# Wenyuan-Vincent-Li/Tensorflow-Implementation-of-Triple-GAN

Measured on AMD Instinct MI355X. Metric: Triple-GAN train images/sec (G+C+D step) CIFAR-10 32x32 bs=100, higher is better.
Workload: dtype f32; 1 GPU; CIFAR-10 32x32x3, 4000 labelled, bs=100 fp32 (B_G/L_C/U_C/L_D/U_D=100/50/50/20/80), Good_GAN_cifar10 D+G+C step; global_batch=100, parallelism=dp1, exec_mode=auto, exec_mode_chosen=plan, hip_graph=False

## Files before the change

### include/tg_kernels.h

```cpp
#ifndef TG_KERNELS_H
#define TG_KERNELS_H

#include <stdint.h>

#ifdef __cplusplus
extern "C" {
#endif

typedef enum tg_status {
  TG_OK = 0,
  TG_ERR_INVALID = -1,
  TG_ERR_HIP = -2,
  TG_ERR_STATE = -3
} tg_status;

enum { TG_ACT_NONE = 0, TG_ACT_LRELU = 1, TG_ACT_RELU = 2, TG_ACT_TANH = 3, TG_ACT_SIGMOID = 4, TG_ACT_SOFTPLUS = 5 };

int tg_version(void);
const char* tg_last_error_string(void);
int tg_device_count(void);

int tg_graph_begin_capture(void* stream);
int tg_graph_end_capture(void* stream, void** graph_exec_out);
int tg_graph_launch(void* graph_exec, void* stream);
// ... 71 lines not shown

int tg_conv3x3_packed_supported(int n, int h, int w, int c_in, int c_out);
int64_t tg_conv3x3_packed_wgrad_workspace_bytes(int n, int h, int w, int c_in, int c_out);
int tg_conv3x3_packed_fwd_f32(const float* x, int ld_x, int c_in, const float* kernel, const float* bias, int act, float alpha, const float* labels,
                              int lab_n, float* y, int ld_y, int n, int h, int w, int c_out, void* stream);
int tg_conv3x3_packed_wgrad_f32(const float* x, int ld_x, int c_in, const float* dy, int ld_dy, int n, int h, int w, int c_out, float* workspace,
                                float* dw, void* stream);

int tg_deconv5x5s2_narrow_supported(int n, int h, int w, int c_out, int ci_p);
int64_t tg_deconv5x5s2_narrow_wgrad_workspace_bytes(int n, int h, int w, int c_out, int ci_p);
int tg_deconv5x5s2_narrow_dgrad_f32(const float* dy, int ld_dy, const float* kernel, const float* scale_a, int n, int h, int w, int c_out, int c_in,
                                    int ci_p, float* dx, int ld_dx, void* stream);
int tg_deconv5x5s2_narrow_wgrad_f32(const float* dy, int ld_dy, const float* x, int ld_x, int n, int h, int w, int c_out, int c_in, int ci_p,
                                    float* workspace, float* dw, void* stream);

int tg_conv2d_desc_fwd(int n, int h, int w, int ld_in, int c_out, int k, int stride, int pad_same, int ld_out, int n_store, int act, float alpha,
                       tg_igemm_desc* d);
int tg_conv2d_desc_dgrad(int n, int h, int w, int c_in_pad, int ld_dy, int k, int stride, int pad_same, int ld_out, int n_store, tg_igemm_desc* descs,
                         int32_t* n_desc_out);
int tg_conv2d_desc_wgrad(int n, int h, int w, int ld_in, int c_out_pad, int k, int stride, int pad_same, int ld_dy, tg_igemm_desc* d);
int tg_deconv5x5s2_desc_fwd(int n, int h, int w, int ld_in, int c_out_pad, int ld_out, int n_store, int act, tg_igemm_desc* descs, int32_t* n_desc_out);
int tg_deconv5x5s2_desc_fwd_merged(int n, int h, int w, int ld_in, int c_out, int ld_out, int n_store, int act, tg_igemm_desc* d, int32_t* n_group_out,
                                   int32_t* tapmap);
int tg_deconv5x5s2_desc_dgrad(int n, int h, int w, int c_in_pad, int ld_dy, int ld_out, int n_store, tg_igemm_desc* d);
int tg_deconv5x5s2_desc_wgrad(int n, int h, int w, int ld_dy, int c_in_pad, int ld_x, tg_igemm_desc* d);
int tg_dense_desc(int m, int ld_in, int c_out, int ld_out, int n_store, int act, int64_t w_sn, tg_igemm_desc* d);
int tg_dense_splitk_desc(int m, int k_dim, int n_out, int splits, tg_igemm_desc* descs);
int tg_wgrad_splits(const tg_igemm_desc* d);
int tg_wgrad_splits_bf16(const tg_igemm_desc* d);
int64_t tg_wgrad_workspace_bytes(const tg_igemm_desc* d, int n_split);
int64_t tg_filter_workspace_bytes(int n_taps, int c_in_pad, int c_out_pad);
int tg_igemm_tile(const tg_igemm_desc* descs, int n_desc, const int32_t* seg_rows, int nseg, int bf16, int32_t* bm_out, int32_t* bn_out);
int tg_igemm_colsum_supported(const tg_igemm_desc* d, const int32_t* seg_rows, int nseg);
int tg_wgrad_tile(const tg_igemm_desc* d, int32_t* ct_out, int32_t* nt_out);

int tg_conv3x3_policy(int policy);
int64_t tg_conv3x3_launches(void);

int tg_wn_scale_f32(const float* v, const float* g, int rows, int c, float* scale, void* stream);

int tg_filter_prep_f32(const float* src, const float* scale, const float* scale_a, int t, int a, int b, int a_pad, int b_pad, float* dst_same,
                       float* dst_tr, int64_t tr_sb, int64_t tr_st, void* stream);

int tg_wn_scale_tab_f32(const float* v, const float* g, int t, int a, int b, float* scale_a, void* stream);
int tg_wn_bwd_tab_f32(const float* dw, const float* v, const float* g, int t, int a, int b, float* dv, float* dg, void* stream);

int tg_deconv_merge_prep_f32(const float* w, const float* scale_a, int c_out, int c_in, int n_group, int n_pad, int c_pad,
                             const int32_t* tapmap, float* dst, void* stream);
typedef struct tg_prep_job {
  const float* src;
  const float* g;
  float* scale;
  float* dst_same;
  float* dst_tr;
  int64_t tr_sb, tr_st;
  int32_t t, a, b, a_pad, b_pad;
} tg_prep_job;
int tg_filter_prep_multi_f32(const tg_prep_job* jobs, int n_jobs, void* stream);
typedef struct tg_wn_job {
  const float* slab;
  float* dw;
  const float* v;
  const float* g;
  float* dv;
  float* dg;
  float* coef;
// ... 181 lines not shown
```

### tensorflow-implementation-of-triple-gan_amd/csrc/geom.cpp

```cpp
#include <cstring>

#include "tg_common.h"
#include "tg_geom.h"
#include "tg_conv3x3_bf16.h"

namespace {

inline int pad32(int c) { return (c + 31) / 32 * 32; }

struct Pad { int out, before; };

Pad same_pad(int n, int k, int s) {
  const int out = (n + s - 1) / s;
  int total = (out - 1) * s + k - n;
  if (total < 0) total = 0;
  return {out, total / 2};
}

Pad out_size(int n, int k, int s, int pad_same) { return pad_same ? same_pad(n, k, s) : Pad{(n - k) / s + 1, 0}; }

struct Tap { int dy, dx, tw; };

int fill(tg_igemm_desc* d, int n_img, int h_in, int w_in, int ld_in, int h_v, int w_v, int s, int h_out, int w_out, int ld_out, int os, int oo_y,
         int oo_x, int c_out, int n_store, const Tap* taps, int n_taps, int64_t w_sn, int64_t w_st, int act, float alpha) {
// ... 88 lines not shown
    int shortest = nk[0];
    for (int s = 1; s < n_sub; ++s) shortest = nk[s] < shortest ? nk[s] : shortest;
    for (;;) {
      int longest = 0, ls = -1, sum = 0;
      for (int s = 0; s < n_sub; ++s) {
        sum += best_ks[s];
        const int len = (nk[s] + best_ks[s] - 1) / best_ks[s];
        if (len > longest) { longest = len; ls = s; }
      }
      if (ls < 0 || best_ks[ls] >= 4 || T * (sum + 1) > slots || sum + 1 > 16) break;
      if (nk[ls] / (best_ks[ls] + 1) < mink || longest * 4 <= shortest * 5) break;
      ++best_ks[ls];
    }
  }
  int len = 0, nslot = 0, nsp = 0;
  for (int s = 0; s < n_sub; ++s) {
    o->ks[s] = best_ks[s];
    if (best_ks[s] > 1) { o->split_sub[nsp] = (int8_t)s; o->first_slot[nsp] = (int8_t)nslot; ++nsp; }
    for (int k = 0; k < best_ks[s]; ++k) {
      o->pat_sub[len] = (int8_t)s; o->pat_k[len] = (int8_t)k;
      o->pat_slot[len] = best_ks[s] > 1 ? (int8_t)nslot++ : (int8_t)-1;
      ++len;
    }
  }
  o->pat_len = len;
  o->n_pat_split = nslot;
  o->n_split_sub = nsp;
  o->nfull = (int)T;
  o->n_units = (int)(T * len);
  o->n_fix = (int)(T * nsp);
  o->ws_bytes = T * nslot * (int64_t)bm * bn * 4;
}

int wgrad_tile(int n) { return n % 128 == 0 ? 128 : ((n % 64 == 0 || n >= 160) ? 64 : 32); }

}

extern "C" {

int tg_conv2d_desc_fwd(int n, int h, int w, int ld_in, int c_out, int k, int stride, int pad_same, int ld_out, int n_store, int act, float alpha,
                       tg_igemm_desc* d) {
  GEOM_ARGS_OK(d && n > 0 && h > 0 && w > 0 && k >= 1 && k <= 5 && stride >= 1 && (pad_same || (h >= k && w >= k)), "conv2d_desc_fwd: bad arguments");
  const Pad py = out_size(h, k, stride, pad_same), px = out_size(w, k, stride, pad_same);
  Tap taps[TG_MAX_TAPS];
  int nt = 0;
  for (int ky = 0; ky < k; ++ky)
    for (int kx = 0; kx < k; ++kx) taps[nt++] = {ky - py.before, kx - px.before, ky * k + kx};
  if (ld_out <= 0) ld_out = c_out;
  if (n_store < 0) n_store = c_out;
  return fill(d, n, h, w, ld_in, py.out, px.out, stride, py.out, px.out, ld_out, 1, 0, 0, c_out, n_store, taps, nt, (int64_t)k * k * ld_in, ld_in, act, alpha);
}

int tg_conv2d_desc_dgrad(int n, int h, int w, int c_in_pad, int ld_dy, int k, int stride, int pad_same, int ld_out, int n_store, tg_igemm_desc* descs,
                         int32_t* n_desc_out) {
  GEOM_ARGS_OK(descs && n_desc_out && n > 0 && h > 0 && w > 0 && k >= 1 && k <= 5 && stride >= 1 && stride <= 2, "conv2d_desc_dgrad: bad arguments");
  const Pad py = out_size(h, k, stride, pad_same), px = out_size(w, k, stride, pad_same);
  if (ld_out <= 0) ld_out = c_in_pad;
  if (n_store < 0) n_store = c_in_pad;
  int nd = 0;
  for (int qy = 0; qy < stride; ++qy)
    for (int qx = 0; qx < stride; ++qx) {
      Tap taps[TG_MAX_TAPS];
      int nt = 0;
      for (int ky = 0; ky < k; ++ky) {
        if (((qy + py.before - ky) % stride + stride) % stride) continue;
        for (int kx = 0; kx < k; ++kx) {
// ... 114 lines not shown
  const int ct = tg::wgrad_tile(d->ld_in), nt = tg::wgrad_tile(d->c_out);
  const int64_t tiles = (int64_t)d->n_taps * ((d->ld_in + ct - 1) / ct) * ((d->c_out + nt - 1) / nt);
  const int64_t m = (int64_t)d->n_img * d->h_v * d->w_v;
  int64_t ns = 512 / tiles;
  if (ns > m / 128) ns = m / 128;
  return (int)(ns < 1 ? 1 : ns);
}

int tg_wgrad_splits_bf16(const tg_igemm_desc* d) {
  if (!d || d->ld_in <= 0 || d->c_out <= 0 || d->n_taps <= 0) { tg::set_error("wgrad_splits_bf16: bad descriptor"); return TG_ERR_INVALID; }
  const int ns = tg::wgrad3x3_splits(d, true, tg::halo_policy(), tg::halo_compute_units());
  return ns > 0 ? ns : tg_wgrad_splits(d);
}

int64_t tg_wgrad_workspace_bytes(const tg_igemm_desc* d, int n_split) {
  if (!d || n_split < 1) { tg::set_error("wgrad_workspace_bytes: bad arguments"); return TG_ERR_INVALID; }
  return (int64_t)n_split * d->n_taps * d->ld_in * d->c_out * 4;
}

int64_t tg_filter_workspace_bytes(int n_taps, int c_in_pad, int c_out_pad) {
  if (n_taps < 1 || c_in_pad < 1 || c_out_pad < 1) { tg::set_error("filter_workspace_bytes: bad arguments"); return TG_ERR_INVALID; }
  return (int64_t)n_taps * c_in_pad * c_out_pad * 4;
}

int tg_igemm_tile(const tg_igemm_desc* descs, int n_desc, const int32_t* seg_rows, int nseg, int bf16, int32_t* bm_out, int32_t* bn_out) {
  TG_REQUIRE(descs && n_desc >= 1 && n_desc <= 4 && bm_out && bn_out, "igemm_tile: bad arguments");
  int bm = 0, bn = 0;
  TG_REQUIRE(tg::igemm_pick_tile(descs, n_desc, nseg > 0, seg_rows, nseg, bf16 != 0, &bm, &bn), "igemm_tile: no tile fits c_out=%d with the given segments",
             descs[0].c_out);
  *bm_out = bm; *bn_out = bn;
  return TG_OK;
}

int tg_wgrad_tile(const tg_igemm_desc* d, int32_t* ct_out, int32_t* nt_out) {
  TG_REQUIRE(d && ct_out && nt_out && d->ld_in > 0 && d->c_out > 0, "wgrad_tile: bad arguments");
  *ct_out = tg::wgrad_tile(d->ld_in);
  *nt_out = tg::wgrad_tile(d->c_out);
  return TG_OK;
}

int tg_igemm_colsum_supported(const tg_igemm_desc* d, const int32_t* seg_rows, int nseg) {
  if (!d || !seg_rows || nseg < 1 || nseg > 8 || d->n_group != 0) return 0;
  int64_t tot = 0;
  for (int i = 0; i < nseg; ++i) { if (seg_rows[i] < 32) return 0; tot += seg_rows[i]; }
  if (tot != (int64_t)d->n_img * d->h_v * d->w_v) return 0;
  int bm, bn;
  return tg::igemm_pick_tile(d, 1, true, seg_rows, nseg, false, &bm, &bn) ? 1 : 0;
}

}
```

### tensorflow-implementation-of-triple-gan_amd/csrc/igemm.hip

```cpp
#include <cstdio>
#include <cstring>
#include "tg_common.h"
#include "tg_device.h"
#include "tg_geom.h"
#include "tg_conv3x3_bf16.h"

typedef float f32x4 __attribute__((ext_vector_type(4)));
typedef float f32x16 __attribute__((ext_vector_type(16)));
typedef __bf16 bf16x8 __attribute__((ext_vector_type(8)));

namespace {

__device__ __forceinline__ bf16x8 cvt8(f32x4 lo, f32x4 hi) {
  bf16x8 r;
  r[0] = (__bf16)lo[0]; r[1] = (__bf16)lo[1]; r[2] = (__bf16)lo[2]; r[3] = (__bf16)lo[3];
  r[4] = (__bf16)hi[0]; r[5] = (__bf16)hi[1]; r[6] = (__bf16)hi[2]; r[7] = (__bf16)hi[3];
  return r;
}

typedef short s16x4 __attribute__((ext_vector_type(4)));
typedef __bf16 bf16x4_t __attribute__((ext_vector_type(4)));
typedef unsigned int u32x2 __attribute__((ext_vector_type(2)));
typedef unsigned int u32x4 __attribute__((ext_vector_type(4)));

// ... 26 lines not shown
  float alpha;
  int32_t n_group;
  int32_t taps[TG_MAX_TAPS];
};

struct IgemmParams {
  const float* in;
  const float* w;
  const float* bias;
  float* out;
  SubDesc d[MAX_SUB];
  int64_t w_sn, w_st;
  int n_img, h_in, w_in, ld_in, c_out;
  int n_sub, M, m_tiles, n_tiles;
  uint32_t in_bytes, w_bytes, out_bytes;
  double* colsum;
  const float* ymul;
  int ymul_act;
  float ymul_alpha;
  int stat2;
  int nseg, seg_rows[8];
  const float* lab;
  int lab_n, lab_c0;
  int n_units;
  int n_fix;
  int nfull;
  int ks[MAX_SUB];
  int pat_len;
  int n_pat_split;
  int n_split_sub;
  int8_t pat_sub[16], pat_k[16], pat_slot[16];
  int8_t split_sub[MAX_SUB], first_slot[MAX_SUB];
  float* ws;
};


__device__ __forceinline__ float apply_act(float v, int act, float alpha) {
  switch (act) {
    case TG_ACT_LRELU: return v > 0.f ? v : alpha * v;
    case TG_ACT_RELU: return v > 0.f ? v : 0.f;
    case TG_ACT_TANH: return tanhf(v);
    case TG_ACT_SIGMOID: return 1.f / (1.f + __expf(-v));
    case TG_ACT_SOFTPLUS: return v > 20.f ? v : log1pf(__expf(v));
    default: return v;
  }
}

__device__ __forceinline__ int xcd_remap(int bid, int nwg) {
  const int q = nwg >> 3, r = nwg & 7, x = bid & 7;
  return (x < r ? x * (q + 1) : r * (q + 1) + (x - r) * q) + (bid >> 3);
}

template <int BM, int BN, int WAVES_M, int WAVES_N, bool COLSUM, bool BF16, bool FIXUP = false>
__global__ void __launch_bounds__(256, 2) igemm_f32_kernel(IgemmParams p) {
  static_assert(WAVES_M * WAVES_N == 4, "4 waves");
  constexpr int WM = BM / WAVES_M, WN = BN / WAVES_N, MI = WM / 32, NI = WN / 32;
  constexpr int AR = BM / 32, BR = BN / 32;
  constexpr int NBUF = 2;
  constexpr int PF = FIXUP ? 1 : (BM * BN >= 128 * 128 ? 1 : 2);
  __shared__ __attribute__((aligned(16))) float smem[NBUF * BM * LDT + NBUF * BN * LDT + 4 * BM];
  float* As = smem;
  float* Bs = smem + NBUF * BM * LDT;
  int* t_base = reinterpret_cast<int*>(smem + NBUF * BM * LDT + NBUF * BN * LDT);
  int* t_y = t_base + BM;
  int* t_x = t_y + BM;
  int* t_out = t_x + BM;

  const int tid = threadIdx.x, lane = tid & 63, wave = tid >> 6;
#ifdef TG_STAMP
  unsigned long long t_entry = 0;
  STAMP(t_entry);
  const unsigned long long rt0 = __builtin_amdgcn_s_memrealtime();
#endif
  int sub, rem_id, kseg = 0, kcut = 1, slot = -1;
  if constexpr (FIXUP) {
    if (p.pat_len > 0) {
      rem_id = blockIdx.x / p.n_split_sub;
      const int j = blockIdx.x - rem_id * p.n_split_sub;
      sub = p.split_sub[j];
      slot = rem_id * p.n_pat_split + p.first_slot[j];
    } else {
      sub = 0;
      rem_id = p.nfull + blockIdx.x;
      slot = blockIdx.x * p.ks[0];
    }
    kcut = p.ks[sub];
  } else {
    const int lid = xcd_remap(blockIdx.x, p.n_units);
    if (p.pat_len > 0) {
      const int L = p.pat_len;
      rem_id = lid / L;
      const int w = (32 % L == 0) ? (lid + (lid >> 5)) % L : lid - rem_id * L;
      sub = p.pat_sub[w]; kseg = p.pat_k[w]; kcut = p.ks[sub];
      slot = p.pat_slot[w] < 0 ? -1 : rem_id * p.n_pat_split + p.pat_slot[w];
    } else {
      sub = 0;
      if (lid < p.nfull) rem_id = lid;
      else {
        const int v = lid - p.nfull;
        kcut = p.ks[0];
        rem_id = p.nfull + v / kcut;
        kseg = v - (rem_id - p.nfull) * kcut;
        slot = v;
      }
    }
  }
  const SubDesc& d = p.d[sub];
  const int nt = rem_id % p.n_tiles, mt = rem_id / p.n_tiles;
  const int m0 = mt * BM, n0 = nt * BN;

  if (tid < BM) {
    int m = m0 + tid;
    int base = 0, y0 = -30000, x0 = 0, oo = (int)0x80000000;
    if (m < p.M) {
      int hw = d.h_v * d.w_v;
      int img = m / hw, rem = m - img * hw;
      int vy = rem / d.w_v, vx = rem - vy * d.w_v;
      base = img * p.h_in * p.w_in * p.ld_in;
      y0 = vy * d.s_y;
      x0 = vx * d.s_x;
      oo = ((img * d.h_out + vy * d.os_y + d.oo_y) * d.w_out + vx * d.os_x + d.oo_x) * d.ld_out * 4;
    }
    t_base[tid] = base; t_y[tid] = y0; t_x[tid] = x0; t_out[tid] = oo;
  }
  __syncthreads();

  const int seg = tid & 7, lrow = tid >> 3;
  int abase[AR], ay[AR], ax[AR];
#pragma unroll
  for (int j = 0; j < AR; ++j) {
    int r = lrow + 32 * j;
    abase[j] = t_base[r] + seg * 4; ay[j] = t_y[r]; ax[j] = t_x[r];
  }

  const __amdgpu_buffer_rsrc_t rsrc = __builtin_amdgcn_make_buffer_rsrc(const_cast<float*>(p.in), 0, p.in_bytes, 0x00020000);
  const __amdgpu_buffer_rsrc_t rsrc_w = __builtin_amdgcn_make_buffer_rsrc(const_cast<float*>(p.w), 0, p.w_bytes, 0x00020000);
  uint32_t wvoff[BR];
#pragma unroll
  for (int j = 0; j < BR; ++j) wvoff[j] = (uint32_t)(((int64_t)(n0 + lrow + 32 * j) * p.w_sn + seg * 4) * 4);

  u32x4 ra[PF][AR], rb[PF][BR];
  uint32_t avoff[AR];
  const int cchunks = p.ld_in / BK;
  const int nk = d.n_taps * cchunks;
  const int h_in = p.h_in, w_in = p.w_in, ld_in = p.ld_in;
  int w_tap_off = 0;

  auto set_tap = [&](int tap) {
    const int tp = d.taps[tap];
    const int dy = (int)(int8_t)(tp >> 8), dx = (int)(int8_t)tp;
    w_tap_off = (tp >> 16) * (int)p.w_st;
#pragma unroll
    for (int j = 0; j < AR; ++j) {
      const int iy = ay[j] + dy, ix = ax[j] + dx;
      const bool ok = (unsigned)iy < (unsigned)h_in && (unsigned)ix < (unsigned)w_in;
      avoff[j] = ok ? (uint32_t)(abase[j] + (iy * w_in + ix) * ld_in) * 4u : OOB_OFF;
    }
  };
  auto gload = [&](int c0, int rs) {
    const uint32_t sa = (uint32_t)__builtin_amdgcn_readfirstlane(c0 * 4);
    const uint32_t sw = (uint32_t)__builtin_amdgcn_readfirstlane((w_tap_off + c0) * 4);
#pragma unroll
    for (int j = 0; j < AR; ++j) ra[rs][j] = __builtin_amdgcn_raw_buffer_load_b128(rsrc, avoff[j], sa, 0);
#pragma unroll
    for (int j = 0; j < BR; ++j) rb[rs][j] = __builtin_amdgcn_raw_buffer_load_b128(rsrc_w, wvoff[j], sw, 0);
  };
  auto sstore = [&](int buf, int rs) {
    if constexpr (BF16) {
      unsigned char* a = reinterpret_cast<unsigned char*>(As) + (buf * BM + lrow) * LDH + seg * 8;
      unsigned char* b = reinterpret_cast<unsigned char*>(Bs) + (buf * BN + lrow) * LDH + seg * 8;
#pragma unroll
      for (int j = 0; j < AR; ++j) *reinterpret_cast<u32x2*>(a + 32 * j * LDH) = pack4_bf16(ra[rs][j]);
#pragma unroll
      for (int j = 0; j < BR; ++j) *reinterpret_cast<u32x2*>(b + 32 * j * LDH) = pack4_bf16(rb[rs][j]);
    } else {
      float* a = As + buf * BM * LDT + lrow * LDT + seg * 4;
      float* b = Bs + buf * BN * LDT + lrow * LDT + seg * 4;
#pragma unroll
// ... 1 lines not shown
#pragma unroll
      for (int j = 0; j < BR; ++j) *reinterpret_cast<u32x4*>(b + 32 * j * LDT) = rb[rs][j];
    }
  };

  const int wm0 = (wave / WAVES_N) * WM, wn0 = (wave % WAVES_N) * WN;
  f32x16 acc[MI][NI];
#pragma unroll
  for (int mi = 0; mi < MI; ++mi)
#pragma unroll
    for (int ni = 0; ni < NI; ++ni)
#pragma unroll
      for (int r = 0; r < 16; ++r) acc[mi][ni][r] = 0.f;

  const int frag = (lane & 31) * LDT + (lane >> 5) * 4;
  constexpr int WS_VEC = MI * NI * 4;

  if constexpr (FIXUP) {
    for (int k = 0; k < kcut; ++k) {
      const f32x4* src = reinterpret_cast<const f32x4*>(p.ws) + ((int64_t)(slot + k) * WS_VEC) * 256 + tid;
#pragma unroll
      for (int mi = 0; mi < MI; ++mi)
#pragma unroll
        for (int ni = 0; ni < NI; ++ni)
#pragma unroll
          for (int q = 0; q < 4; ++q) {
            const f32x4 v = src[((mi * NI + ni) * 4 + q) * 256];
            acc[mi][ni][4 * q] += v[0]; acc[mi][ni][4 * q + 1] += v[1]; acc[mi][ni][4 * q + 2] += v[2]; acc[mi][ni][4 * q + 3] += v[3];
          }
    }
  } else {
  const int it0 = (int)((int64_t)nk * kseg / kcut), it1 = (int)((int64_t)nk * (kseg + 1) / kcut);

  int tap = it0 / cchunks, c0 = (it0 - tap * cchunks) * BK, buf = 0, issued = it0;
  set_tap(tap);
  auto issue = [&](int rs) {
    gload(c0, rs);
    ++issued;
    c0 += BK;
    if (c0 == ld_in) { c0 = 0; ++tap; if (issued < it1) set_tap(tap); }
  };
#ifdef TG_STAMP
  unsigned long long ts0 = 0, ts1 = 0, ts2 = 0, ts3 = 0, ts4 = 0, acc_load = 0, acc_mfma = 0, acc_store = 0, acc_bar = 0, t_begin = 0;
#endif
#pragma unroll
  for (int rs = 0; rs < PF; ++rs)
    if (it0 + rs < it1) issue(rs);
  sstore(0, 0);
  __syncthreads();

#ifdef TG_STAMP
  STAMP(t_begin);
#endif
  auto compute = [&](int b) {
    if constexpr (BF16) {
      const unsigned char* Ab = reinterpret_cast<const unsigned char*>(As) + (b * BM + wm0 + (lane & 31)) * LDH + (lane >> 5) * 16;
      const unsigned char* Bb = reinterpret_cast<const unsigned char*>(Bs) + (b * BN + wn0 + (lane & 31)) * LDH + (lane >> 5) * 16;
#pragma unroll
      for (int G = 0; G < BK / 16; ++G) {
        bf16x8 fa[MI], fb[NI];
#pragma unroll
        for (int mi = 0; mi < MI; ++mi) fa[mi] = *reinterpret_cast<const bf16x8*>(Ab + mi * 32 * LDH + G * 32);
#pragma unroll
        for (int ni = 0; ni < NI; ++ni) fb[ni] = *reinterpret_cast<const bf16x8*>(Bb + ni * 32 * LDH + G * 32);
#pragma unroll
        for (int mi = 0; mi < MI; ++mi)
#pragma unroll
          for (int ni = 0; ni < NI; ++ni)
            if (COLSUM) acc[mi][ni] = __builtin_amdgcn_mfma_f32_32x32x16_bf16(fa[mi], fb[ni], acc[mi][ni], 0, 0, 0);
            else acc[mi][ni] = __builtin_amdgcn_mfma_f32_32x32x16_bf16(fb[ni], fa[mi], acc[mi][ni], 0, 0, 0);
      }
    } else {
      const float* A = As + b * BM * LDT + wm0 * LDT + frag;
// ... 28 lines not shown
      float* wa = As + (buf ^ 1) * BM * LDT + lrow * LDT + seg * 4;
      float* wb = Bs + (buf ^ 1) * BN * LDT + lrow * LDT + seg * 4;
      f32x4 fa[2], fb[2];
      fa[0] = *reinterpret_cast<const f32x4*>(A);
      fb[0] = *reinterpret_cast<const f32x4*>(B);
      __builtin_amdgcn_sched_barrier(0);
#pragma unroll
      for (int k = 0; k < 16; ++k) {
        const int g = k >> 2, sft = k & 3, cur = g & 1;
        if (COLSUM) acc[0][0] = __builtin_amdgcn_mfma_f32_32x32x2f32(fa[cur][sft], fb[cur][sft], acc[0][0], 0, 0, 0);
        else acc[0][0] = __builtin_amdgcn_mfma_f32_32x32x2f32(fb[cur][sft], fa[cur][sft], acc[0][0], 0, 0, 0);
        if (sft == 0 && g < 3) fa[cur ^ 1] = *reinterpret_cast<const f32x4*>(A + (g + 1) * 8);
        else if (sft == 1 && g < 3) fb[cur ^ 1] = *reinterpret_cast<const f32x4*>(B + (g + 1) * 8);
        else {
          const int j = (g < 3) ? 2 * g + (sft - 2) : 6 + sft;
          if (j < NL) {
            if (do_load) {
              if (j < AR) ra[rs][j < AR ? j : 0] = __builtin_amdgcn_raw_buffer_load_b128(rsrc, avoff[j < AR ? j : 0], sa, 0);
              else rb[rs][j >= AR ? j - AR : 0] = __builtin_amdgcn_raw_buffer_load_b128(rsrc_w, wvoff[j >= AR ? j - AR : 0], sw, 0);
            }
          } else if (j < 2 * NL) {
            const int q = j - NL;
            if (do_write) {
              if (q < AR) *reinterpret_cast<u32x4*>(wa + 32 * (q < AR ? q : 0) * LDT) = ra[ws][q < AR ? q : 0];
              else *reinterpret_cast<u32x4*>(wb + 32 * (q >= AR ? q - AR : 0) * LDT) = rb[ws][q >= AR ? q - AR : 0];
            }
          }
        }
        __builtin_amdgcn_sched_barrier(0);
      }
      if (do_load) {
        ++issued;
        c0 += BK;
        if (c0 == ld_in) { c0 = 0; ++tap; if (issued < it1) set_tap(tap); }
      }
      __syncthreads();
      buf ^= 1;
    };
    while (issued + PF <= it1) {
#pragma unroll
      for (int rs = 0; rs < PF; ++rs) ktile(rs, true, true);
      it += PF;
    }
    for (; it < it1; it += PF) {
#pragma unroll
      for (int rs = 0; rs < PF; ++rs)
        if (it + rs < it1) ktile(rs, issued < it1, it + rs + 1 < it1);
    }
  }
  while (issued + PF <= it1) {
#pragma unroll
    for (int rs = 0; rs < PF; ++rs) {
      STAMP(ts0);
      issue(rs);
      STAMP(ts1);
      compute(buf);
      STAMP(ts2);
      sstore(buf ^ 1, (rs + 1) % PF);
      STAMP(ts3);
      __syncthreads();
      STAMP(ts4);
#ifdef TG_STAMP
      acc_load += ts1 - ts0; acc_mfma += ts2 - ts1; acc_store += ts3 - ts2; acc_bar += ts4 - ts3;
#endif
      buf ^= 1;
    }
    it += PF;
// ... 620 lines not shown
    const tg_igemm_desc& e = descs[order[i]];
    TG_REQUIRE(e.n_img == d->n_img && e.h_v == d->h_v && e.w_v == d->w_v && e.c_out == d->c_out && e.ld_in == d->ld_in && e.h_in == d->h_in &&
               e.w_in == d->w_in && e.w_sn == d->w_sn && e.w_st == d->w_st, "igemm: sub-problem %d differs in M / N / gathered tensor / filter strides", i);
    SubDesc& k = p.d[i];
    k.h_v = e.h_v; k.w_v = e.w_v; k.s_y = e.s_y; k.s_x = e.s_x; k.h_out = e.h_out; k.w_out = e.w_out; k.ld_out = e.ld_out;
    k.os_y = e.os_y; k.os_x = e.os_x; k.oo_y = e.oo_y; k.oo_x = e.oo_x; k.n_store = e.n_store; k.n_taps = e.n_taps; k.act = e.act;
    k.alpha = e.alpha;
    k.n_group = e.n_group;
    for (int t = 0; t < e.n_taps; ++t)
      k.taps[t] = ((int32_t)e.tapw[t] << 16) | (((int32_t)e.dy[t] & 0xff) << 8) | ((int32_t)e.dx[t] & 0xff);
  }
  p.w_sn = d->w_sn; p.w_st = d->w_st;
  p.n_img = d->n_img; p.h_in = d->h_in; p.w_in = d->w_in; p.ld_in = d->ld_in; p.c_out = d->c_out;
  p.M = d->n_img * d->h_v * d->w_v;
  const int64_t in_bytes = (int64_t)d->n_img * d->h_in * d->w_in * d->ld_in * 4;
  TG_REQUIRE(in_bytes < 0x7FFFFFF0LL, "igemm: gathered tensor exceeds the 2 GiB buffer-descriptor range");
  p.in_bytes = (uint32_t)in_bytes;
  int max_tapw = 0;
  for (int i = 0; i < n_desc; ++i)
    for (int t = 0; t < descs[i].n_taps; ++t) max_tapw = descs[i].tapw[t] > max_tapw ? descs[i].tapw[t] : max_tapw;
  const int64_t w_bytes = ((int64_t)(d->c_out - 1) * d->w_sn + (int64_t)max_tapw * d->w_st + d->ld_in) * 4;
  TG_REQUIRE(w_bytes > 0 && w_bytes < 0x7FFFFFF0LL && d->w_st >= 0 && d->w_sn >= 0 && (int64_t)max_tapw * d->w_st < 0x7FFFFFFFLL,
             "igemm: filter extent outside the 2 GiB buffer-descriptor range");
  p.w_bytes = (uint32_t)w_bytes;
  int64_t out_bytes = 0;
  for (int i = 0; i < n_desc; ++i) {
    const int64_t ob = (int64_t)descs[i].n_img * descs[i].h_out * descs[i].w_out * descs[i].ld_out * 4;
    out_bytes = ob > out_bytes ? ob : out_bytes;
  }
  TG_REQUIRE(out_bytes < 0x7FFFFFF0LL, "igemm: output tensor exceeds the 2 GiB buffer-descriptor range");
  p.out_bytes = (uint32_t)out_bytes;
  double taps = 0;
  for (int i = 0; i < n_desc; ++i) taps += descs[i].n_taps;
  const double flops = 2.0 * p.M * d->c_out * taps * d->ld_in;
  const double bytes = (in16 ? 2.0 : 4.0) * p.M * d->ld_in + 4.0 * ((double)p.M * d->n_store * n_desc + (double)d->c_out * taps * d->ld_in);
  hipStream_t s = tg::as_stream(stream);
  const bool halo = !lab && tg::conv3x3_bf16_applicable(descs, n_desc, seg_rows, colsum ? nseg : 0, bf16);
  int bm = 0, bn = 0;
  tg::IgemmSched sc;
  std::memset(&sc, 0, sizeof sc);
  if (!halo) {
    TG_REQUIRE(tg::igemm_pick_tile(descs, n_desc, colsum != nullptr, seg_rows, nseg, bf16, &bm, &bn), "igemm: no tile fits c_out=%d with the given segments",
               d->c_out);
    p.m_tiles = (p.M + bm - 1) / bm;
    p.n_tiles = (p.c_out + bn - 1) / bn;
    int nk[MAX_SUB] = {0, 0, 0, 0};
    for (int i = 0; i < n_desc; ++i) nk[i] = descs[order[i]].n_taps * (d->ld_in / BK);
    tg::igemm_schedule(n_desc, nk, (int64_t)p.m_tiles * p.n_tiles, bm, bn, 2 * tg::halo_compute_units(), scratch != nullptr, &sc);
    if (sc.ws_bytes > scratch_bytes || (reinterpret_cast<uintptr_t>(scratch) & 15))
      tg::igemm_schedule(n_desc, nk, (int64_t)p.m_tiles * p.n_tiles, bm, bn, 2 * tg::halo_compute_units(), false, &sc);
  }
  char desc[128];
  snprintf(desc, sizeof(desc), "M=%dx%d N=%d K=%gx%d in=%dx%d s=%d os=%d%s tile=%dx%d units=%d fix=%d ks=%d/%d/%d/%d", n_desc, p.M, d->c_out, taps, d->ld_in, d->h_in,
           d->w_in, d->s_y, d->os_y, bf16 ? " bf16" : "", bm, bn, sc.n_units, sc.n_fix, sc.ks[0], sc.ks[1], sc.ks[2], sc.ks[3]);
  tg::ProfScope prof(tg::PC_IGEMM, flops, bytes, s, desc);
  if (halo)
    return tg::conv3x3_bf16_launch(d, in, w, bias, out, colsum, seg_rows, nseg, ymul, ymul_act, ymul_alpha, in16 ? p.in_bytes / 2 : p.in_bytes, p.w_bytes,
                                   p.out_bytes, s, bf16, scratch, scratch_bytes, stat2, in16);
  p.n_units = sc.n_units; p.n_fix = sc.n_fix; p.nfull = sc.nfull; p.pat_len = sc.pat_len; p.n_pat_split = sc.n_pat_split; p.n_split_sub = sc.n_split_sub;
  for (int i = 0; i < MAX_SUB; ++i) { p.ks[i] = sc.ks[i]; p.split_sub[i] = sc.split_sub[i]; p.first_slot[i] = sc.first_slot[i]; }
  for (int i = 0; i < 16; ++i) { p.pat_sub[i] = sc.pat_sub[i]; p.pat_k[i] = sc.pat_k[i]; p.pat_slot[i] = sc.pat_slot[i]; }
  p.ws = static_cast<float*>(scratch);
  if (bm == 128 && bn == 128) launch_igemm<128, 128, 2, 2>(p, s, bf16);
  else if (bm == 64 && bn == 128) launch_igemm<64, 128, 2, 2>(p, s, bf16);
  else if (bm == 64 && bn == 64) launch_igemm<64, 64, 2, 2>(p, s, bf16);
  else if (bm == 32 && bn == 128) launch_igemm<32, 128, 1, 4>(p, s, bf16);
  else launch_igemm<128, 32, 4, 1>(p, s, bf16);
  TG_CHECK_LAUNCH("igemm_f32_kernel");
  return TG_OK;
}

#ifdef TG_STAMP
extern "C" int tg_debug_read_block_times(unsigned long long* out, int n) {
  hipError_t e = hipMemcpyFromSymbol(out, HIP_SYMBOL(tg_block_times), sizeof(unsigned long long) * 3 * n);
  return e == hipSuccess ? 0 : -2;
}

extern "C" int tg_debug_read_stamps(unsigned long long* out) {
  hipError_t e = hipMemcpyFromSymbol(out, HIP_SYMBOL(tg_stamps), sizeof(unsigned long long) * 64);
  return e == hipSuccess ? 0 : -2;
}
#endif

extern "C" int tg_igemm_multi_f32(const tg_igemm_desc* descs, int n_desc, const float* in, const float* w, const float* bias, float* out,
                                  void* scratch, int64_t scratch_bytes, void* stream) {
  return igemm_impl(descs, n_desc, in, w, bias, out, stream, nullptr, nullptr, 0, false, nullptr, 0, 0.f, scratch, scratch_bytes);
}

extern "C" int tg_igemm_f32(const tg_igemm_desc* d, const float* in, const float* w, const float* bias, float* out, void* scratch,
                            int64_t scratch_bytes, void* stream) {
  return igemm_impl(d, 1, in, w, bias, out, stream, nullptr, nullptr, 0, false, nullptr, 0, 0.f, scratch, scratch_bytes);
}

extern "C" int tg_igemm_labels_f32(const tg_igemm_desc* d, const float* in, const float* w, const float* bias, const float* labels, int n_labels, float* out,
                                   void* scratch, int64_t scratch_bytes, void* stream) {
  TG_REQUIRE(labels != nullptr, "igemm_labels: null labels");
  return igemm_impl(d, 1, in, w, bias, out, stream, nullptr, nullptr, 0, false, nullptr, 0, 0.f, scratch, scratch_bytes, 0, labels, n_labels);
}

extern "C" int tg_igemm_labels_bf16(const tg_igemm_desc* d, const float* in, const float* w, const float* bias, const float* labels, int n_labels, float* out,
                                    void* scratch, int64_t scratch_bytes, void* stream) {
  TG_REQUIRE(labels != nullptr, "igemm_labels: null labels");
  return igemm_impl(d, 1, in, w, bias, out, stream, nullptr, nullptr, 0, true, nullptr, 0, 0.f, scratch, scratch_bytes, 0, labels, n_labels);
}

static int64_t igemm_ws_bytes(const tg_igemm_desc* descs, int n_desc, const int32_t* seg_rows, int nseg, bool bf16, bool in16 = false) {
  const bool colsum = nseg > 0;
  HeadTail ht;
  if (head_tail(descs, n_desc, seg_rows, nseg, colsum, bf16, &ht)) {
    const int64_t a = igemm_ws_bytes(&ht.dh, 1, colsum ? ht.seg_h : nullptr, ht.nh, bf16, in16);
    const int64_t b = igemm_ws_bytes(&ht.dt, 1, colsum ? ht.seg_t : nullptr, ht.nt, bf16, in16);
    return a > b ? a : b;
  }
  if (tg::conv3x3_bf16_applicable(descs, n_desc, seg_rows, colsum ? nseg : 0, bf16)) return bf16 ? tg::conv3x3_bf16_pack_bytes(descs, n_desc) : 0;
  if (in16) return widen_bytes(&descs[0]) + igemm_ws_bytes(descs, n_desc, seg_rows, nseg, bf16, false);
  int bm = 0, bn = 0;
  if (!tg::igemm_pick_tile(descs, n_desc, colsum, seg_rows, nseg, bf16, &bm, &bn)) return 0;
  int order[MAX_SUB] = {0, 1, 2, 3}, nk[MAX_SUB] = {0, 0, 0, 0};
  tg::igemm_sub_order(descs, n_desc, order);
  for (int i = 0; i < n_desc; ++i) nk[i] = descs[order[i]].n_taps * (descs[0].ld_in / BK);
  const int64_t M = (int64_t)descs[0].n_img * descs[0].h_v * descs[0].w_v;
  tg::IgemmSched sc;
  tg::igemm_schedule(n_desc, nk, ((M + bm - 1) / bm) * ((descs[0].c_out + bn - 1) / bn), bm, bn, 2 * tg::halo_compute_units(), true, &sc);
  return sc.ws_bytes;
}

extern "C" int64_t tg_igemm_workspace_bytes(const tg_igemm_desc* descs, int n_desc, const int32_t* seg_rows, int nseg, int bf16) {
  if (!descs || n_desc < 1 || n_desc > MAX_SUB || nseg < 0 || nseg > 8 || (nseg > 0 && !seg_rows)) { tg::set_error("igemm_workspace_bytes: bad arguments"); return TG_ERR_INVALID; }
  for (int i = 0; i < n_desc; ++i)
    if (descs[i].ld_in <= 0 || descs[i].c_out <= 0 || descs[i].n_taps <= 0 || descs[i].n_taps > TG_MAX_TAPS || descs[i].n_img <= 0) { tg::set_error("igemm_workspace_bytes: bad descriptor"); return TG_ERR_INVALID; }
  return igemm_ws_bytes(descs, n_desc, seg_rows, nseg, bf16 != 0, bf16 == 2);
}

static int igemm_colsum_impl(const tg_igemm_desc* d, const float* in, const float* w, float* out, const int32_t* seg_rows, int nseg,
                             double* colsum, int colsum_zeroed, void* stream, bool bf16, const float* ymul = nullptr, int ymul_act = 0,
                             float ymul_alpha = 0.f, void* scratch = nullptr, int64_t scratch_bytes = 0) {
  TG_REQUIRE(d && colsum && seg_rows && nseg >= 1 && nseg <= 8, "igemm_colsum: bad args");
  TG_REQUIRE(d->n_group == 0, "igemm_colsum: grouped columns are not supported");
  TG_REQUIRE(d->act == TG_ACT_NONE, "igemm_colsum: the statistics are of the raw convolution output (no activation)");
  int tot = 0;
  for (int i = 0; i < nseg; ++i) { TG_REQUIRE(seg_rows[i] >= 32, "igemm_colsum: segment %d has %d rows (need at least one 32-row tile)", i, seg_rows[i]); tot += seg_rows[i]; }
  TG_REQUIRE(tot == d->n_img * d->h_v * d->w_v, "igemm_colsum: segments sum to %d rows, launch has %d", tot, d->n_img * d->h_v * d->w_v);
  if (!colsum_zeroed) {
    hipError_t e = hipMemsetAsync(colsum, 0, sizeof(double) * nseg * d->c_out, tg::as_stream(stream));
    if (e != hipSuccess) return tg::hip_fail(e, "hipMemsetAsync(colsum)");
  }
  return igemm_impl(d, 1, in, w, nullptr, out, stream, colsum, seg_rows, nseg, bf16, ymul, ymul_act, ymul_alpha, scratch, scratch_bytes);
}

extern "C" int tg_igemm_colsum_f32(const tg_igemm_desc* d, const float* in, const float* w, float* out, const int32_t* seg_rows, int nseg,
// ... 181 lines not shown
```

### tensorflow-implementation-of-triple-gan_amd/csrc/tg_geom.h

```cpp
#pragma once
#include <stdint.h>
#include "../../include/tg_kernels.h"

namespace tg {

bool igemm_pick_tile(const tg_igemm_desc* descs, int n_desc, bool colsum, const int32_t* seg_rows, int nseg, bool bf16, int* bm_out, int* bn_out);
struct IgemmSched {
  int n_units, n_fix, nfull, ks[4], pat_len, n_pat_split, n_split_sub;
  int8_t pat_sub[16], pat_k[16], pat_slot[16], split_sub[4], first_slot[4];
  int64_t ws_bytes;
};
void igemm_schedule(int n_sub, const int* nk, int64_t tiles, int bm, int bn, int slots, bool allow_split, IgemmSched* out);
void igemm_sub_order(const tg_igemm_desc* descs, int n_desc, int* order);
int wgrad_tile(int n);

}
```

### tensorflow-implementation-of-triple-gan_amd/tg/geom.py

```python
import ctypes as C

from . import lib
from .lib import ACT, IgemmDesc


def pad32(c):
    return (c + 31) // 32 * 32


def _same(padding):
    if padding not in ('SAME', 'VALID'):
        raise ValueError("padding must be 'SAME' or 'VALID', got %r" % (padding,))
    return 1 if padding == 'SAME' else 0


def _opt(v, neg=False):
    return (-1 if neg else 0) if v is None else int(v)


def _many(fn, *args):
    arr = (IgemmDesc * 4)()
    n = C.c_int32()
    lib.call(fn, *args, C.cast(arr, C.c_void_p), C.byref(n))
    return [arr[i] for i in range(n.value)]
# ... 29 lines not shown
    d = IgemmDesc()
    lib.call('tg_deconv5x5s2_desc_dgrad', n, h, w, c_in_pad, ld_dy, _opt(ld_out), _opt(n_store, True), C.byref(d))
    return d


def deconv_wgrad(n, h, w, ld_dy, c_in_pad, ld_x=None):
    d = IgemmDesc()
    lib.call('tg_deconv5x5s2_desc_wgrad', n, h, w, ld_dy, c_in_pad, _opt(ld_x), C.byref(d))
    return d


def dense_fwd(m, ld_in, c_out, ld_out=None, n_store=None, act=None, w_sn=None):
    d = IgemmDesc()
    lib.call('tg_dense_desc', m, ld_in, c_out, _opt(ld_out), _opt(n_store, True), ACT[act], _opt(w_sn), C.byref(d))
    return d


def dense_fwd_splitk(m, k_dim, n_out, splits):
    arr = (IgemmDesc * 4)()
    lib.call('tg_dense_splitk_desc', m, k_dim, n_out, splits, C.cast(arr, C.c_void_p))
    return [arr[i] for i in range(splits)]


def wgrad_splits(desc, bf16=False):
    return lib.call('tg_wgrad_splits_bf16' if bf16 else 'tg_wgrad_splits', C.byref(desc))


def wgrad_slab_floats(desc, n_split):
    return lib.call('tg_wgrad_workspace_bytes', C.byref(desc), n_split) // 4


def colsum_supported(desc, seg_rows):
    return bool(lib.call('tg_igemm_colsum_supported', C.byref(desc), (C.c_int32 * len(seg_rows))(*seg_rows), len(seg_rows)))
```

Baseline: 7209 images/sec.

## Add position-class igemm tiling that skips out-of-bounds padding taps

Adds a 'posclass' mode to the implicit-GEMM conv kernel for stride-1 convolutions with spatial padding and small output maps. M-tiles are grouped by output position, so each tile covers images at one position and iterates only the taps that land in bounds, selected through a per-tile bitmask. Positions are sorted by tap count so heavy tiles are scheduled first. The aim is to remove MFMA work and loads spent on zero-padded taps in small-spatial layers. In exchange it drops split-K scheduling for those layers and can launch more, smaller tiles when the batch does not fill BM, and a heuristic picks between the two paths.

```diff
diff --git a/include/tg_kernels.h b/include/tg_kernels.h
--- a/include/tg_kernels.h
+++ b/include/tg_kernels.h
@@ -127,6 +127,8 @@
 int64_t tg_filter_workspace_bytes(int n_taps, int c_in_pad, int c_out_pad);
 int tg_igemm_tile(const tg_igemm_desc* descs, int n_desc, const int32_t* seg_rows, int nseg, int bf16, int32_t* bm_out, int32_t* bn_out);
 int tg_igemm_colsum_supported(const tg_igemm_desc* d, const int32_t* seg_rows, int nseg);
+int tg_igemm_route(const tg_igemm_desc* descs, int n_desc, const int32_t* seg_rows, int nseg, int bf16, int32_t* route_out);
+int tg_igemm_posclass_policy(int policy, int32_t* was_out);
 int tg_wgrad_tile(const tg_igemm_desc* d, int32_t* ct_out, int32_t* nt_out);
 
 int tg_conv3x3_policy(int policy);
diff --git a/tensorflow-implementation-of-triple-gan_amd/csrc/geom.cpp b/tensorflow-implementation-of-triple-gan_amd/csrc/geom.cpp
--- a/tensorflow-implementation-of-triple-gan_amd/csrc/geom.cpp
+++ b/tensorflow-implementation-of-triple-gan_amd/csrc/geom.cpp
@@ -144,6 +144,33 @@
   o->ws_bytes = T * nslot * (int64_t)bm * bn * 4;
 }
 
+int g_posclass_policy = 0;
+
+bool igemm_posclass(const tg_igemm_desc* descs, int n_desc, bool colsum, bool labels, int bm, IgemmPosClass* o) {
+  const tg_igemm_desc* d = &descs[0];
+  if (g_posclass_policy == 2 || n_desc != 1 || colsum || labels || d->n_group != 0 || d->s_y != 1 || d->s_x != 1 || bm < 1) return false;
+  if (!(d->h_in < d->h_v || d->w_in < d->w_v) || d->h_v * d->w_v > PC_MAX_POS || d->n_taps > 31) return false;
+  std::memset(o, 0, sizeof *o);
+  o->n_pos = d->h_v * d->w_v;
+  for (int pos = 0; pos < o->n_pos; ++pos) {
+    const int vy = pos / d->w_v, vx = pos % d->w_v;
+    int nt = 0;
+    for (int t = 0; t < d->n_taps; ++t) {
+      const int iy = vy + d->dy[t], ix = vx + d->dx[t];
+      nt += (iy >= 0 && iy < d->h_in && ix >= 0 && ix < d->w_in) ? 1 : 0;
+    }
+    o->taps_total += nt;
+    int i = pos;
+    for (; i > 0 && o->ntap[i - 1] < nt; --i) { o->pos[i] = o->pos[i - 1]; o->ntap[i] = o->ntap[i - 1]; }
+    o->pos[i] = (uint8_t)pos; o->ntap[i] = (uint8_t)nt;
+  }
+  o->tpp = (d->n_img + bm - 1) / bm;
+  o->m_tiles = o->n_pos * o->tpp;
+  if (g_posclass_policy == 1) return true;
+  const int64_t M = (int64_t)d->n_img * o->n_pos;
+  return (int64_t)o->tpp * o->taps_total < ((M + bm - 1) / bm) * d->n_taps;
+}
+
 int wgrad_tile(int n) { return n % 128 == 0 ? 128 : ((n % 64 == 0 || n >= 160) ? 64 : 32); }
 
 }
@@ -324,6 +351,22 @@
   return TG_OK;
 }
 
+int tg_igemm_route(const tg_igemm_desc* descs, int n_desc, const int32_t* seg_rows, int nseg, int bf16, int32_t* route_out) {
+  TG_REQUIRE(descs && n_desc >= 1 && n_desc <= 4 && route_out, "igemm_route: bad arguments");
+  int bm = 0, bn = 0;
+  TG_REQUIRE(tg::igemm_pick_tile(descs, n_desc, nseg > 0, seg_rows, nseg, bf16 != 0, &bm, &bn), "igemm_route: no tile fits c_out=%d with the given segments",
+             descs[0].c_out);
+  tg::IgemmPosClass pc;
+  *route_out = tg::igemm_posclass(descs, n_desc, nseg > 0, false, bm, &pc) ? 1 : 0;
+  return TG_OK;
+}
+
+int tg_igemm_posclass_policy(int policy, int32_t* was_out) {
+  if (was_out) *was_out = tg::g_posclass_policy;
+  if (policy >= 0 && policy <= 2) tg::g_posclass_policy = policy;
+  return TG_OK;
+}
+
 int tg_wgrad_tile(const tg_igemm_desc* d, int32_t* ct_out, int32_t* nt_out) {
   TG_REQUIRE(d && ct_out && nt_out && d->ld_in > 0 && d->c_out > 0, "wgrad_tile: bad arguments");
   *ct_out = tg::wgrad_tile(d->ld_in);
diff --git a/tensorflow-implementation-of-triple-gan_amd/csrc/igemm.hip b/tensorflow-implementation-of-triple-gan_amd/csrc/igemm.hip
--- a/tensorflow-implementation-of-triple-gan_amd/csrc/igemm.hip
+++ b/tensorflow-implementation-of-triple-gan_amd/csrc/igemm.hip
@@ -82,6 +82,8 @@
   int8_t pat_sub[16], pat_k[16], pat_slot[16];
   int8_t split_sub[MAX_SUB], first_slot[MAX_SUB];
   float* ws;
+  int pc_tpp, pc_mtiles;
+  uint8_t pc_pos[tg::PC_MAX_POS];
 };
 
 
@@ -122,8 +124,22 @@
   STAMP(t_entry);
   const unsigned long long rt0 = __builtin_amdgcn_s_memrealtime();
 #endif
-  int sub, rem_id, kseg = 0, kcut = 1, slot = -1;
-  if constexpr (FIXUP) {
+  int sub, rem_id = 0, kseg = 0, kcut = 1, slot = -1;
+  int pc_pos = -1, pc_img0 = 0;
+  if constexpr (!FIXUP) {
+    if (p.pc_tpp > 0) {
+      const int x = blockIdx.x & 7, j = blockIdx.x >> 3;
+      const int mi = (j / p.n_tiles) * 8 + x;
+      if (mi >= p.pc_mtiles) return;
+      const int pr = mi / p.pc_tpp;
+      pc_pos = p.pc_pos[pr];
+      pc_img0 = (mi - pr * p.pc_tpp) * BM;
+      rem_id = mi * p.n_tiles + (j % p.n_tiles);
+    }
+  }
+  if (pc_pos >= 0) {
+    sub = 0;
+  } else if constexpr (FIXUP) {
     if (p.pat_len > 0) {
       rem_id = blockIdx.x / p.n_split_sub;
       const int j = blockIdx.x - rem_id * p.n_split_sub;
@@ -162,9 +178,11 @@
   if (tid < BM) {
     int m = m0 + tid;
     int base = 0, y0 = -30000, x0 = 0, oo = (int)0x80000000;
-    if (m < p.M) {
-      int hw = d.h_v * d.w_v;
-      int img = m / hw, rem = m - img * hw;
+    int hw = d.h_v * d.w_v;
+    int img = m / hw, rem = m - img * hw;
+    bool live = m < p.M;
+    if (pc_pos >= 0) { img = pc_img0 + tid; rem = pc_pos; live = img < p.n_img; }
+    if (live) {
       int vy = rem / d.w_v, vx = rem - vy * d.w_v;
       base = img * p.h_in * p.w_in * p.ld_in;
       y0 = vy * d.s_y;
@@ -192,8 +210,19 @@
   u32x4 ra[PF][AR], rb[PF][BR];
   uint32_t avoff[AR];
   const int cchunks = p.ld_in / BK;
-  const int nk = d.n_taps * cchunks;
   const int h_in = p.h_in, w_in = p.w_in, ld_in = p.ld_in;
+  uint32_t tmask = (1u << d.n_taps) - 1u;
+  if (pc_pos >= 0) {
+    const int vy = pc_pos / d.w_v, vx = pc_pos - vy * d.w_v;
+    tmask = 0;
+    for (int t = 0; t < d.n_taps; ++t) {
+      const int tp = d.taps[t];
+      const int iy = vy * d.s_y + (int)(int8_t)(tp >> 8), ix = vx * d.s_x + (int)(int8_t)tp;
+      if ((unsigned)iy < (unsigned)h_in && (unsigned)ix < (unsigned)w_in) tmask |= 1u << t;
+    }
+  }
+  tmask = (uint32_t)__builtin_amdgcn_readfirstlane((int)tmask);
+  const int nk = __builtin_popcount(tmask) * cchunks;
   int w_tap_off = 0;
 
   auto set_tap = [&](int tap) {
@@ -261,13 +290,21 @@
   } else {
   const int it0 = (int)((int64_t)nk * kseg / kcut), it1 = (int)((int64_t)nk * (kseg + 1) / kcut);
 
-  int tap = it0 / cchunks, c0 = (it0 - tap * cchunks) * BK, buf = 0, issued = it0;
-  set_tap(tap);
+  const int tap0 = it0 / cchunks;
+  for (int i = 0; i < tap0; ++i) tmask &= tmask - 1u;
+  int tap = __builtin_ctz(tmask | 0x80000000u), c0 = (it0 - tap0 * cchunks) * BK, buf = 0, issued = it0;
+  if (it0 < it1) set_tap(tap);
+  auto next_tap = [&]() {
+    c0 = 0;
+    tmask &= tmask - 1u;
+    tap = __builtin_ctz(tmask | 0x80000000u);
+    if (issued < it1) set_tap(tap);
+  };
   auto issue = [&](int rs) {
     gload(c0, rs);
     ++issued;
     c0 += BK;
-    if (c0 == ld_in) { c0 = 0; ++tap; if (issued < it1) set_tap(tap); }
+    if (c0 == ld_in) next_tap();
   };
 #ifdef TG_STAMP
   unsigned long long ts0 = 0, ts1 = 0, ts2 = 0, ts3 = 0, ts4 = 0, acc_load = 0, acc_mfma = 0, acc_store = 0, acc_bar = 0, t_begin = 0;
@@ -362,7 +399,7 @@
       if (do_load) {
         ++issued;
         c0 += BK;
-        if (c0 == ld_in) { c0 = 0; ++tap; if (issued < it1) set_tap(tap); }
+        if (c0 == ld_in) next_tap();
       }
       __syncthreads();
       buf ^= 1;
@@ -1049,13 +1086,17 @@
   p.out_bytes = (uint32_t)out_bytes;
   double taps = 0;
   for (int i = 0; i < n_desc; ++i) taps += descs[i].n_taps;
-  const double flops = 2.0 * p.M * d->c_out * taps * d->ld_in;
+  double flops = 2.0 * p.M * d->c_out * taps * d->ld_in;
   const double bytes = (in16 ? 2.0 : 4.0) * p.M * d->ld_in + 4.0 * ((double)p.M * d->n_store * n_desc + (double)d->c_out * taps * d->ld_in);
   hipStream_t s = tg::as_stream(stream);
   const bool halo = !lab && tg::conv3x3_bf16_applicable(descs, n_desc, seg_rows, colsum ? nseg : 0, bf16);
   int bm = 0, bn = 0;
   tg::IgemmSched sc;
   std::memset(&sc, 0, sizeof sc);
+  tg::IgemmPosClass pc;
+  bool posclass = false;
+  p.pc_tpp = 0; p.pc_mtiles = 0;
+  std::memset(p.pc_pos, 0, sizeof p.pc_pos);
   if (!halo) {
     TG_REQUIRE(tg::igemm_pick_tile(descs, n_desc, colsum != nullptr, seg_rows, nseg, bf16, &bm, &bn), "igemm: no tile fits c_out=%d with the given segments",
                d->c_out);
@@ -1063,13 +1104,24 @@
     p.n_tiles = (p.c_out + bn - 1) / bn;
     int nk[MAX_SUB] = {0, 0, 0, 0};
     for (int i = 0; i < n_desc; ++i) nk[i] = descs[order[i]].n_taps * (d->ld_in / BK);
-    tg::igemm_schedule(n_desc, nk, (int64_t)p.m_tiles * p.n_tiles, bm, bn, 2 * tg::halo_compute_units(), scratch != nullptr, &sc);
-    if (sc.ws_bytes > scratch_bytes || (reinterpret_cast<uintptr_t>(scratch) & 15))
-      tg::igemm_schedule(n_desc, nk, (int64_t)p.m_tiles * p.n_tiles, bm, bn, 2 * tg::halo_compute_units(), false, &sc);
+    posclass = tg::igemm_posclass(descs, n_desc, colsum != nullptr, lab != nullptr, bm, &pc);
+    if (posclass) {
+      p.pc_tpp = pc.tpp; p.pc_mtiles = pc.m_tiles;
+      std::memcpy(p.pc_pos, pc.pos, sizeof p.pc_pos);
+      p.m_tiles = pc.m_tiles;
+      for (int s_ = 0; s_ < 4; ++s_) sc.ks[s_] = 1;
+      sc.n_units = (pc.m_tiles + 7) / 8 * 8 * p.n_tiles;
+      sc.nfull = sc.n_units;
+      flops = 2.0 * d->n_img * pc.taps_total * d->c_out * d->ld_in;
+    } else {
+      tg::igemm_schedule(n_desc, nk, (int64_t)p.m_tiles * p.n_tiles, bm, bn, 2 * tg::halo_compute_units(), scratch != nullptr, &sc);
+      if (sc.ws_bytes > scratch_bytes || (reinterpret_cast<uintptr_t>(scratch) & 15))
+        tg::igemm_schedule(n_desc, nk, (int64_t)p.m_tiles * p.n_tiles, bm, bn, 2 * tg::halo_compute_units(), false, &sc);
+    }
   }
   char desc[128];
   snprintf(desc, sizeof(desc), "M=%dx%d N=%d K=%gx%d in=%dx%d s=%d os=%d%s tile=%dx%d units=%d fix=%d ks=%d/%d/%d/%d", n_desc, p.M, d->c_out, taps, d->ld_in, d->h_in,
-           d->w_in, d->s_y, d->os_y, bf16 ? " bf16" : "", bm, bn, sc.n_units, sc.n_fix, sc.ks[0], sc.ks[1], sc.ks[2], sc.ks[3]);
+           d->w_in, d->s_y, d->os_y, bf16 ? (posclass ? " bf16 posclass" : " bf16") : (posclass ? " posclass" : ""), bm, bn, sc.n_units, sc.n_fix, sc.ks[0], sc.ks[1], sc.ks[2], sc.ks[3]);
   tg::ProfScope prof(tg::PC_IGEMM, flops, bytes, s, desc);
   if (halo)
     return tg::conv3x3_bf16_launch(d, in, w, bias, out, colsum, seg_rows, nseg, ymul, ymul_act, ymul_alpha, in16 ? p.in_bytes / 2 : p.in_bytes, p.w_bytes,
@@ -1133,6 +1185,8 @@
   if (in16) return widen_bytes(&descs[0]) + igemm_ws_bytes(descs, n_desc, seg_rows, nseg, bf16, false);
   int bm = 0, bn = 0;
   if (!tg::igemm_pick_tile(descs, n_desc, colsum, seg_rows, nseg, bf16, &bm, &bn)) return 0;
+  tg::IgemmPosClass pc;
+  if (tg::igemm_posclass(descs, n_desc, colsum, false, bm, &pc)) return 0;
   int order[MAX_SUB] = {0, 1, 2, 3}, nk[MAX_SUB] = {0, 0, 0, 0};
   tg::igemm_sub_order(descs, n_desc, order);
   for (int i = 0; i < n_desc; ++i) nk[i] = descs[order[i]].n_taps * (descs[0].ld_in / BK);
diff --git a/tensorflow-implementation-of-triple-gan_amd/csrc/tg_geom.h b/tensorflow-implementation-of-triple-gan_amd/csrc/tg_geom.h
--- a/tensorflow-implementation-of-triple-gan_amd/csrc/tg_geom.h
+++ b/tensorflow-implementation-of-triple-gan_amd/csrc/tg_geom.h
@@ -11,6 +11,13 @@
   int64_t ws_bytes;
 };
 void igemm_schedule(int n_sub, const int* nk, int64_t tiles, int bm, int bn, int slots, bool allow_split, IgemmSched* out);
+constexpr int PC_MAX_POS = 64;
+struct IgemmPosClass {
+  int n_pos, tpp, m_tiles;
+  int taps_total;
+  uint8_t pos[PC_MAX_POS], ntap[PC_MAX_POS];
+};
+bool igemm_posclass(const tg_igemm_desc* descs, int n_desc, bool colsum, bool labels, int bm, IgemmPosClass* out);
 void igemm_sub_order(const tg_igemm_desc* descs, int n_desc, int* order);
 int wgrad_tile(int n);
 
diff --git a/tensorflow-implementation-of-triple-gan_amd/tg/geom.py b/tensorflow-implementation-of-triple-gan_amd/tg/geom.py
--- a/tensorflow-implementation-of-triple-gan_amd/tg/geom.py
+++ b/tensorflow-implementation-of-triple-gan_amd/tg/geom.py
@@ -85,3 +85,17 @@
 
 def colsum_supported(desc, seg_rows):
     return bool(lib.call('tg_igemm_colsum_supported', C.byref(desc), (C.c_int32 * len(seg_rows))(*seg_rows), len(seg_rows)))
+
+
+def igemm_route(descs, seg_rows=None, bf16=False):
+    descs = descs if isinstance(descs, (list, tuple)) else [descs]
+    seg = (C.c_int32 * len(seg_rows))(*seg_rows) if seg_rows else None
+    r = C.c_int32()
+    lib.call('tg_igemm_route', C.cast(lib.desc_array(descs), C.c_void_p), len(descs), seg, len(seg_rows) if seg_rows else 0, int(bf16), C.byref(r))
+    return ('dense', 'posclass')[r.value]
+
+
+def posclass_policy(policy=-1):
+    was = C.c_int32()
+    lib.call('tg_igemm_posclass_policy', int(policy), C.byref(was))
+    return was.value
```

Result: no change. 7234 images/sec, median of 6 (+0.4%).
